# manikya7022/Continual-Learning-for-Dynamic-Video-Quality-Enhancement

Hardware: AMD Instinct MI355X
Metric: train frames/sec (2x SR, T=3, 540p->1080p) (higher is better)
Workload: dtype bf16

## Files before the change

### continual-learning-for-dynamic-video-quality-enhancement_amd/csrc/conv_bf16.hip

```cpp
#include "conv_common.h"

namespace nvq {

#ifdef NVQ_DEBUG_TOOLS
static int g_debug_mode = 0;
void set_conv_debug_mode(int m) { g_debug_mode = m; }
#else
constexpr int g_debug_mode = 0;
#endif

constexpr int XSB = 48;

__device__ __forceinline__ __bf16 pack_bf16_elem(const float* __restrict__ w, int cout_w, int cin_w, int taps, int transpose,
                                                 int cout_keep, int NT, int nkc, long idx) {
    const int stride = ws_stride_halfs(taps, NT);
    long t = idx % stride;
    const long slab = idx / stride;
    if (t >= (long)taps * 4 * NT * 8) return (__bf16)0.f;
    const int j = t & 7; t >>= 3;
    const int n = t % NT; t /= NT;
    const int g = t & 3; t >>= 2;
    const int tap = (int)t;
    const int kc = slab % nkc;
    const int cz = (int)(slab / nkc);
// ... 651 lines not shown
#pragma unroll
                for (int xh = 0; xh < 2; ++xh) {
#pragma unroll
                    for (int cb = 0; cb < NB; ++cb)
                        acc[cb][xh] = __builtin_amdgcn_mfma_f32_16x16x32_bf16(wa[cb], lo[xh], acc[cb][xh], 0, 0, 0);
                    if (same_dx) nhi[xh] = ldP(dy + 2, xh, ndx);
                    else if (!last) nlo[xh] = ldP(0, xh, ndx);
                }
#pragma unroll
                for (int xh = 0; xh < 2; ++xh) {
#pragma unroll
                    for (int cb = 0; cb < NB; ++cb)
                        acc[cb][2 + xh] = __builtin_amdgcn_mfma_f32_16x16x32_bf16(wa[cb], hi[xh], acc[cb][2 + xh], 0, 0, 0);
                    if (same_dx) nlo[xh] = hi[xh];
                    else if (!last) nhi[xh] = ldP(1, xh, ndx);
                }
                if (!last) {
#pragma unroll
                    for (int xh = 0; xh < 2; ++xh) { lo[xh] = nlo[xh]; hi[xh] = nhi[xh]; }
#pragma unroll
                    for (int cb = 0; cb < NB; ++cb) wa[cb] = wn[cb];
                }
            }
        }
        __syncthreads();
        reinterpret_cast<u32x4*>(wl)[rtid] = lr;
        __bf16* t4 = ws;
        if (!(dbg & 32)) conv_epilogue<NB>(d3, acc, n, ty, tx, 0, w4, c, g, vec3, TH, t4 + w4 * (2 * TW * T4S));
        __syncthreads();
        if (!(dbg & 32)) {
            __bf16* o16 = reinterpret_cast<__bf16*>(d3.out);
            const __bf16* stage = t4 + w4 * (2 * TW * T4S);
#pragma unroll
            for (int k = 0; k < 4; ++k) {
                const int item = lane + k * 64;
                const int px = item >> 2, piece = item & 3;
                const int gy = ty * TH + 2 * w4 + (px >> 5), gx = tx * TW + (px & 31);
                if (gy < H && gx < W)
                    *reinterpret_cast<u32x4*>(o16 + ((size_t)(n * H + gy) * W + gx) * d3.out_ld + d3.out_coff + 8 * piece) =
                        *reinterpret_cast<const u32x4*>(stage + px * T4S + 8 * piece);
            }
        }
        __syncthreads();
        return;
    }
    f32x4 lacc[NBL][4];
#pragma unroll
    for (int b = 0; b < 4; ++b)
#pragma unroll
        for (int a = 0; a < NBL; ++a) lacc[a][b] = (f32x4){0.f, 0.f, 0.f, 0.f};
    unsigned xoff[XPER];
    bool xok[XPER];
#pragma unroll
    for (int k = 0; k < XPER; ++k) xoff[k] = halo_off(rtid + k * 256, xok[k]);
    u32x4 xr[XPER];
    auto fetch = [&](int kc) {
        int sh;
        const unsigned o0 = chunk_off(kc, sh);
#pragma unroll
        for (int k = 0; k < XPER; ++k) xr[k] = *reinterpret_cast<const u32x4*>(in16 + ((xoff[k] << sh) + o0));
    };
    auto ldL = [&](int cb) -> bf16x8 {
        return *reinterpret_cast<const bf16x8*>(wl + (g * NTL + cb * 16 + c) * 8);
    };
    if (!(dbg & 64)) fetch(0);
    for (int kc = 0; kc < nkc; ++kc) {
        __syncthreads();
        if (!(dbg & 8)) {
            const u32x4 z = {0u, 0u, 0u, 0u};
#pragma unroll
            for (int k = 0; k < XPER; ++k) {
                const int item = rtid + k * 256;
                *reinterpret_cast<u32x4*>(xs + (item >> 2) * XSB + 8 * (item & 3)) = xok[k] ? xr[k] : z;
            }
        }
        __syncthreads();
        if (kc + 1 < nkc && !(dbg & 4)) fetch(kc + 1);
        if (dbg & 2) continue;
        bf16x8 px[4];
        px[0] = ldP(1, 0, 1); px[1] = ldP(1, 1, 1); px[2] = ldP(2, 0, 1); px[3] = ldP(2, 1, 1);
#pragma unroll
        for (int cb = 0; cb < NBL; ++cb) {
            const bf16x8 wf = ldL(cb);
#pragma unroll
            for (int pb = 0; pb < 4; ++pb)
                lacc[cb][pb] = __builtin_amdgcn_mfma_f32_16x16x32_bf16(wf, px[pb], lacc[cb][pb], 0, 0, 0);
        }
    }
    bool okp[4];
    uint2 rr[4][NBL];
    float4 bb[NBL];
    const __bf16* r16 = reinterpret_cast<const __bf16*>(dl.res) + dl.res_coff;
    auto res_load = [&](int pb) {
        const int gy = ty * TH + 2 * w4 + (pb >> 1), gx = tx * TW + (pb & 1) * 16 + c;
        okp[pb] = gy < H && gx < W;
        const unsigned off = okp[pb] ? ((unsigned)(n * H + gy) * (unsigned)W + gx) * (unsigned)dl.res_ld + 4u * g : 0u;
#pragma unroll
        for (int cb = 0; cb < NBL; ++cb) rr[pb][cb] = *reinterpret_cast<const uint2*>(r16 + (off + cb * 16u));
    };
    if (!(dbg & 128)) { res_load(0); res_load(1); }
    __syncthreads();
    __syncthreads();
    {
        const __bf16* t4 = ws;
#pragma unroll
        for (int cb = 0; cb < NBL; ++cb) {
            const bf16x8 wf = ldL(cb);
#pragma unroll
            for (int pb = 0; pb < 4; ++pb) {
                const int px = (2 * w4 + (pb >> 1)) * TW + (pb & 1) * 16 + c;
                const bf16x8 yf = *reinterpret_cast<const bf16x8*>(t4 + px * T4S + 8 * g);
                lacc[cb][pb] = __builtin_amdgcn_mfma_f32_16x16x32_bf16(wf, yf, lacc[cb][pb], 0, 0, 0);
            }
        }
    }
    if (!(dbg & 128)) { res_load(2); res_load(3); }
#pragma unroll
    for (int cb = 0; cb < NBL; ++cb) bb[cb] = ld4(dl.bias + cb * 16 + 4 * g);
    __syncthreads();
    __bf16* stage = lds + w4 * (2 * TW * STAGE_PX64);
#pragma unroll
    for (int pb = 0; pb < 4; ++pb) {
        if (!okp[pb]) continue;
#pragma unroll
        for (int cb = 0; cb < NBL; ++cb) {
            float v[4] = {lacc[cb][pb][0] + bb[cb].x, lacc[cb][pb][1] + bb[cb].y, lacc[cb][pb][2] + bb[cb].z,
                          lacc[cb][pb][3] + bb[cb].w};
            {
#pragma clang fp contract(off)
                v[0] = v[0] * dl.alpha + __uint_as_float(rr[pb][cb].x << 16);
                v[1] = v[1] * dl.alpha + __uint_as_float(rr[pb][cb].x & 0xffff0000u);
                v[2] = v[2] * dl.alpha + __uint_as_float(rr[pb][cb].y << 16);
                v[3] = v[3] * dl.alpha + __uint_as_float(rr[pb][cb].y & 0xffff0000u);
            }
            *reinterpret_cast<bf16x4*>(stage + ((pb >> 1) * TW + (pb & 1) * 16 + c) * STAGE_PX64 + cb * 16 + 4 * g) =
                (bf16x4){(__bf16)v[0], (__bf16)v[1], (__bf16)v[2], (__bf16)v[3]};
        }
    }
    __builtin_amdgcn_fence(__ATOMIC_RELEASE, "wavefront");
    __builtin_amdgcn_wave_barrier();
    if (dbg & 16) return;
    __bf16* o16 = reinterpret_cast<__bf16*>(dl.out);
#pragma unroll
    for (int k = 0; k < 8; ++k) {
        const int item = lane + k * 64;
        const int px = item >> 3, piece = item & 7;
        const int gy = ty * TH + 2 * w4 + (px >> 5), gx = tx * TW + (px & 31);
        if (gy < H && gx < W)
            *reinterpret_cast<u32x4*>(o16 + ((size_t)(n * H + gy) * W + gx) * dl.out_ld + dl.out_coff + 8 * piece) =
                *reinterpret_cast<const u32x4*>(stage + px * STAGE_PX64 + 8 * piece);
    }
}

template <int KS, bool XB, bool YB, int CIC, int COC = 32>
__global__ __launch_bounds__(256, 2) void wgrad_bf16_kernel(const nvq_wgrad_desc d, int tilesX, int tilesY,
                                                             int ntiles, int nci32, int nco) {
    static_assert(CIC == 32 || (CIC == 64 && XB), "64-channel chunks need bf16 x");
    static_assert(COC == 32 || (COC == 64 && CIC == 64 && YB && KS == 1), "64-co chunks: 1x1, bf16 x and dy");
    constexpr int HALO = KS / 2;
    constexpr int TAPS = KS * KS;
    constexpr int HW_ = TW + 2 * HALO;
    constexpr int HH_ = TH + 2 * HALO;
    constexpr int NPIX = HW_ * HH_;
    constexpr int XSX = CIC == 64 ? 80 : XSB;
    constexpr int XPP = (XB ? 4 : 8) * (CIC / 32);
    constexpr int YSX = COC == 64 ? 80 : XSB;
    constexpr int YPP = (YB ? 4 : 8) * (COC / 32);
    constexpr int XCH = CIC / XPP, YCH = COC / YPP;
    constexpr int XITEMS = NPIX * XPP;
    constexpr int XPER = (XITEMS + 255) / 256;
    constexpr int YPER = TH * TW * YPP / 256;
    constexpr int NCO = (CIC == 64 ? 2 : 1) * (COC / 32);
    __shared__ __attribute__((aligned(16))) __bf16 lds[NPIX * XSX + TH * TW * YSX];
    __bf16* xs = lds;
    __bf16* dys = lds + NPIX * XSX;

    const int tid = threadIdx.x;
    const int lane = tid & 63;
    const int wave = tid >> 6;
    const int r = lane & 15;
    const int g = lane >> 4;
    const int q = r >> 2, p = r & 3;
    const int cib = CIC == 64 ? wave : wave >> 1;
    const int cob0 = CIC == 64 ? 0 : (wave & 1);
    const int cic = blockIdx.y, coc = blockIdx.z;
    const int H = d.h, W = d.w;
    const float* x32 = d.x + d.x_coff;
    const __bf16* x16 = reinterpret_cast<const __bf16*>(d.x) + d.x_coff;
    const float* dy32 = d.dy + d.dy_coff;
    const __bf16* dy16 = reinterpret_cast<const __bf16*>(d.dy) + d.dy_coff;

    f32x4 acc[NCO][TAPS];
#pragma unroll
    for (int a = 0; a < NCO; ++a)
#pragma unroll
        for (int t = 0; t < TAPS; ++t) acc[a][t] = (f32x4){0.f, 0.f, 0.f, 0.f};

    u32x4 xr[XPER], yr[YPER];
    float4 bsumA = make_float4(0.f, 0.f, 0.f, 0.f), bsumB = bsumA;
    const int xq = XCH * (tid & (XPP - 1));
    const int yq = YCH * (tid & (YPP - 1));
    const bool xch_ok = cic * CIC + xq < d.cin;
    const int xch = cic * CIC + xq;
    const bool xlead = !d.x_plane || xch < d.x_ld;
    const unsigned xmul = xlead ? d.x_ld : 32;
    const size_t xbase = xlead ? (size_t)xch : (size_t)(xch >> 5) * d.x_plane + (xch & 31);
    const int ych = coc * COC + yq;
    const bool ych_ok = ych < d.cout;
    unsigned xmask = 0, ymask = 0;
    auto fetch = [&](int tile) {
        int bt = xcd_tile(tile, ntiles);
        const int tx = bt % tilesX; bt /= tilesX;
        const int ty = bt % tilesY;
        const int n = bt / tilesY;
        xmask = 0; ymask = 0;
#pragma unroll
        for (int k = 0; k < XPER; ++k) {
            const int item = tid + k * 256;
            const int hp = item / XPP;
            const int hy = hp / HW_, hx = hp - hy * HW_;
            const int gy = ty * TH + hy - HALO, gx = tx * TW + hx - HALO;
            const bool ok = item < XITEMS && gy >= 0 && gy < H && gx >= 0 && gx < W && xch_ok;
            xmask |= (ok ? 1u : 0u) << k;
            const size_t off = ok ? ((size_t)(n * H + gy) * W + gx) * xmul + xbase : 0;
            if constexpr (XB) xr[k] = *reinterpret_cast<const u32x4*>(x16 + off);
            else xr[k] = *reinterpret_cast<const u32x4*>(x32 + off);
        }
#pragma unroll
        for (int k = 0; k < YPER; ++k) {
            const int item = tid + k * 256;
            const int pp = item / YPP;
            const int py = pp / TW, px = pp - py * TW;
            const int gy = ty * TH + py, gx = tx * TW + px;
            const bool ok = gy < H && gx < W && ych_ok;
            ymask |= (ok ? 1u : 0u) << k;
            const size_t off = ok ? ((size_t)(n * H + gy) * W + gx) * d.dy_ld + ych : 0;
            if constexpr (YB) yr[k] = *reinterpret_cast<const u32x4*>(dy16 + off);
            else yr[k] = *reinterpret_cast<const u32x4*>(dy32 + off);
        }
    };
    auto commit = [&]() {
        const u32x4 z = {0u, 0u, 0u, 0u};
#pragma unroll
        for (int k = 0; k < XPER; ++k) {
            const int item = tid + k * 256;
            if (item < XITEMS) {
                const u32x4 v = (xmask >> k) & 1 ? xr[k] : z;
                __bf16* dst = xs + (item / XPP) * XSX + XCH * (item & (XPP - 1));
                if constexpr (XB) *reinterpret_cast<u32x4*>(dst) = v;
                else *reinterpret_cast<bf16x4*>(dst) = cvt4(as_f4(v));
            }
        }
#pragma unroll
        for (int k = 0; k < YPER; ++k) {
            const int item = tid + k * 256;
            const u32x4 v = (ymask >> k) & 1 ? yr[k] : z;
            __bf16* dst = dys + (item / YPP) * YSX + YCH * (item & (YPP - 1));
            if constexpr (YB) {
                *reinterpret_cast<u32x4*>(dst) = v;
                bsumA.x += bf_lo(v[0]); bsumA.y += bf_hi(v[0]); bsumA.z += bf_lo(v[1]); bsumA.w += bf_hi(v[1]);
                bsumB.x += bf_lo(v[2]); bsumB.y += bf_hi(v[2]); bsumB.z += bf_lo(v[3]); bsumB.w += bf_hi(v[3]);
            } else {
                const float4 f = as_f4(v);
                *reinterpret_cast<bf16x4*>(dst) = cvt4(f);
                bsumA.x += f.x; bsumA.y += f.y; bsumA.z += f.z; bsumA.w += f.w;
            }
        }
    };
    const bool idle = cic * CIC + cib * 16 >= d.cin_w;
    typedef s16x4 __attribute__((address_space(3))) * lds_s16x4_ptr;
    auto tr_read = [&](const __bf16* base, int stride, int pix, int chblock) -> s16x4 {
        return __builtin_amdgcn_ds_read_tr16_b64_v4i16((lds_s16x4_ptr)(base + (pix + q) * stride + chblock * 16 + 4 * p));
    };

    int tile = blockIdx.x;
    if (tile < ntiles) fetch(tile);
    for (; tile < ntiles; tile += gridDim.x) {
        __syncthreads();
        commit();
        __syncthreads();
        if (tile + (int)gridDim.x < ntiles) fetch(tile + gridDim.x);
        if (idle) continue;
#pragma unroll 2
        for (int py = 0; py < TH; ++py) {
            bf16x8 bfrag[NCO];
#pragma unroll
            for (int a = 0; a < NCO; ++a) {
                const s16x4 b0 = tr_read(dys, YSX, py * TW + 4 * g, cob0 + a);
                const s16x4 b1 = tr_read(dys, YSX, py * TW + 16 + 4 * g, cob0 + a);
                bfrag[a] = __builtin_bit_cast(bf16x8, __builtin_shufflevector(b0, b1, 0, 1, 2, 3, 4, 5, 6, 7));
            }
#pragma unroll
            for (int tap = 0; tap < TAPS; ++tap) {
                const int ddy = tap / KS, ddx = tap - ddy * KS;
                const int hp = (py + ddy) * HW_ + ddx;
                const s16x4 a0 = tr_read(xs, XSX, hp + 4 * g, cib);
                const s16x4 a1 = tr_read(xs, XSX, hp + 16 + 4 * g, cib);
                const bf16x8 afrag = __builtin_bit_cast(bf16x8, __builtin_shufflevector(a0, a1, 0, 1, 2, 3, 4, 5, 6, 7));
#pragma unroll
                for (int a = 0; a < NCO; ++a)
                    acc[a][tap] = __builtin_amdgcn_mfma_f32_16x16x32_bf16(afrag, bfrag[a], acc[a][tap], 0, 0, 0);
            }
        }
    }

    const int slab = cic * (CIC / 32) + (cib * 16) / 32;
    if (slab < nci32) {
        const int cil0 = (cib * 16) % 32;
#pragma unroll
        for (int a = 0; a < NCO; ++a) {
            const int coc32 = coc * (COC / 32) + (cob0 + a) / 2, cob = (cob0 + a) % 2;
            if (coc32 >= nco) continue;
            float* part = d.workspace + ((size_t)(blockIdx.x * nci32 + slab) * nco + coc32) * (TAPS * WG_C * WG_C);
#pragma unroll
            for (int tap = 0; tap < TAPS; ++tap)
#pragma unroll
                for (int e = 0; e < 4; ++e) part[(tap * WG_C + cil0 + 4 * g + e) * WG_C + cob * 16 + r] = acc[a][tap][e];
        }
    }

    if (cic == 0 && d.dbias != nullptr) {
        float* scratch = reinterpret_cast<float*>(lds);
        __syncthreads();
        st4(scratch + 8 * tid, bsumA);
        st4(scratch + 8 * tid + 4, bsumB);
        __syncthreads();
        if (tid < COC) {
            const int piece = tid / YCH, e = tid % YCH;
            float s = 0.f;
            for (int k = 0; k < 256 / YPP; ++k) s += scratch[8 * (YPP * k + piece) + e];
            float* bp = d.workspace + (size_t)WGRAD_MAX_SLABS * 9 * WG_C * WG_C;
            const int coc32 = coc * (COC / 32) + tid / WG_C;
            if (coc32 < nco) bp[((size_t)blockIdx.x * nco + coc32) * WG_C + tid % WG_C] = s;
        }
    }
}

size_t pack_floats_bf16(int cout, int cin_store, int ksize) {
    const int NT = choose_nt(cout);
    const size_t ncz = (cout + NT - 1) / NT, nkc = (cin_store + KCB - 1) / KCB;
    return ncz * nkc * (size_t)ws_stride_halfs(ksize * ksize, NT) / 2;
}

int pack_bf16(const float* w, int cout_w, int cin_w, int ksize, int transpose, int cin_store, int cout_keep,
              float* wpack, hipStream_t s) {
    const int cout = transpose ? cout_keep : cout_w;
    const int NT = choose_nt(cout);
    const int ncz = (cout + NT - 1) / NT, nkc = (cin_store + KCB - 1) / KCB;
    const long total = (long)ncz * nkc * ws_stride_halfs(ksize * ksize, NT);
    int nblk = ceil_div(total, 256);
    if (nblk > 2048) nblk = 2048;
    hipLaunchKernelGGL(pack_bf16_kernel, dim3(nblk), dim3(256), 0, s, w, cout_w, cin_w, ksize * ksize, transpose,
                       cout_keep, NT, ncz, nkc, reinterpret_cast<__bf16*>(wpack));
    return check_launch("conv_pack_bf16");
}

PackJobDev pack_job_bf16(const nvq_pack_job& j) {
    const int cout = j.transpose ? j.cout_keep : j.cout_w;
    const int NT = choose_nt(cout);
    const int ncz = (cout + NT - 1) / NT, nkc = (j.cin_store + KCB - 1) / KCB;
    return PackJobDev{j.w, j.wpack, j.cout_w, j.cin_w, j.ksize * j.ksize, j.transpose, j.cout_keep, NT, ncz, nkc,
                      (long)ncz * nkc * ws_stride_halfs(j.ksize * j.ksize, NT)};
}

int pack_batch_bf16(const PackJobTable& t, int n, hipStream_t s) {
    hipLaunchKernelGGL(pack_batch_bf16_kernel, dim3(32, n), dim3(256), 0, s, t);
    return check_launch("conv_pack_batch(bf16)");
}

int conv_forward_bf16(const nvq_conv_desc& d, int vec_ok, hipStream_t s) {
    NVQ_REQUIRE((size_t)d.n * d.h * d.w * d.in_ld < ((size_t)1 << 32),
                "conv_forward(bf16): input tensor of %d x %d x %d x %d elements exceeds the 32-bit offsets of the kernels", d.n,
                d.h, d.w, d.in_ld);
    const int NT = choose_nt(d.cout);
    const int ncz = (d.cout_store + NT - 1) / NT;
    const int nkc = (d.cin + KCB - 1) / KCB;
    int tilesX = (d.w + TW - 1) / TW, tilesY = (d.h + TH - 1) / TH;
    const bool underfilled = tilesX * ((d.h + 2 * TH - 1) / (2 * TH)) < NVQ_SMALL_IMAGE_TILES;
    const int rows = d.tile_rows == 0 && underfilled ? 8 : d.tile_rows;
    if (d.ksize == 3 && NT == 32 && d.in_bf16 && d.h >= 2 * TH && vec_ok &&
        (rows == 162 || rows == 164 || (rows == 0 && d.cin <= 128)))
        return conv_forward_m32(d, rows == 164 ? 4 : 2, g_debug_mode & 15, s);
    if (d.ksize == 3 && NT == 32 && d.in_bf16 && d.h >= 2 * TH && rows != 8) {
        tilesY = (d.h + 2 * TH - 1) / (2 * TH);
        const dim3 grid8((unsigned)((long)tilesX * tilesY * d.n), ncz);
        hipLaunchKernelGGL((conv_bf16_kernel<2, 3, true, 8>), grid8, dim3(512), 0, s, d, tilesX, tilesY, nkc, vec_ok,
                           g_debug_mode & 3, TailArgs{});
        return check_launch("conv_forward_bf16");
    }
    if (d.ksize == 3 && NT == 64 && d.in_bf16 && (d.tile_rows == 264 || d.tile_rows == 265)) {
        NVQ_REQUIRE(vec_ok && d.out_bf16 && d.cout_store % 64 == 0 && d.cin % 8 == 0,
                    "conv_forward: tile_rows 264 / 265 need bf16 output and a multiple of 64 stored channels");
        return conv_forward_m32(d, d.tile_rows == 264 ? 64 : 65, g_debug_mode & 3, s);
    }
    if (d.ksize == 3 && NT == 64 && d.in_bf16 && d.tile_rows != 8) {
        const dim3 grid8((unsigned)((long)tilesX * tilesY * d.n), ncz);
        hipLaunchKernelGGL((conv_bf16_kernel<2, 3, true, 8, 2>), grid8, dim3(512), 0, s, d, tilesX, tilesY, nkc, vec_ok,
                           g_debug_mode & 3, TailArgs{});
        return check_launch("conv_forward_bf16");
    }
    const dim3 grid((unsigned)((long)tilesX * tilesY * d.n), ncz);
#define NVQ_LAUNCH_CONVB(NB, KS)                                                                                        \
    do {                                                                                                                 \
        if (d.in_bf16)                                                                                                   \
            hipLaunchKernelGGL((conv_bf16_kernel<NB, KS, true>), grid, dim3(256), 0, s, d, tilesX, tilesY, nkc, vec_ok, g_debug_mode & 3, TailArgs{});   \
        else                                                                                                             \
            hipLaunchKernelGGL((conv_bf16_kernel<NB, KS, false>), grid, dim3(256), 0, s, d, tilesX, tilesY, nkc, vec_ok, g_debug_mode & 3, TailArgs{});  \
    } while (0)
    if (d.ksize == 3) {
        if (NT == 16) NVQ_LAUNCH_CONVB(1, 3);
        else if (NT == 32) NVQ_LAUNCH_CONVB(2, 3);
        else NVQ_LAUNCH_CONVB(4, 3);
    } else {
        if (NT == 16) NVQ_LAUNCH_CONVB(1, 1);
        else if (NT == 32) NVQ_LAUNCH_CONVB(2, 1);
        else NVQ_LAUNCH_CONVB(4, 1);
    }
#undef NVQ_LAUNCH_CONVB
    return check_launch("conv_forward_bf16");
}

int upsampler_tail_bf16(const nvq_conv_desc& d, const float* frames, int T, int t_center, int Cimg, int s, float* out,
                        unsigned char* pass, hipStream_t st) {
    NVQ_REQUIRE((size_t)d.n * d.h * d.w * d.in_ld < ((size_t)1 << 32), "upsampler_tail: tensor exceeds 32-bit offsets");
    const int tilesX = (d.w + TW - 1) / TW, tilesY = (d.h + TH - 1) / TH;
    const int nkc = (d.cin + KCB - 1) / KCB;
    const dim3 grid((unsigned)((long)tilesX * tilesY * d.n), 1);
    const TailArgs t{frames, out, pass, T, t_center, Cimg};
    if (s == 2 && Cimg * 4 <= 16)
        hipLaunchKernelGGL((conv_bf16_kernel<1, 3, true, 4, 1, 2>), grid, dim3(256), 0, st, d, tilesX, tilesY, nkc, 0, 0, t);
    else if (s == 3 && Cimg * 9 <= 32)
        hipLaunchKernelGGL((conv_bf16_kernel<2, 3, true, 4, 1, 3>), grid, dim3(256), 0, st, d, tilesX, tilesY, nkc, 0, 0, t);
    else if (s == 4 && Cimg * 16 <= 64)
        hipLaunchKernelGGL((conv_bf16_kernel<4, 3, true, 4, 1, 4>), grid, dim3(256), 0, st, d, tilesX, tilesY, nkc, 0, 0, t);
    else
        NVQ_REQUIRE(false, "upsampler_tail: scale %d with %d image channels", s, Cimg);
    return check_launch("upsampler_tail_forward");
}

void conv_occupancy_bf16(int* out) {
    (void)hipOccupancyMaxActiveBlocksPerMultiprocessor(&out[0], conv_bf16_kernel<2, 3, true, 8>, 512, 0);
    (void)hipOccupancyMaxActiveBlocksPerMultiprocessor(&out[1], conv_bf16_kernel<2, 3, true, 8, 2>, 512, 0);
    (void)hipOccupancyMaxActiveBlocksPerMultiprocessor(&out[2], conv_bf16_kernel<4, 3, true, 4>, 256, 0);
    (void)hipOccupancyMaxActiveBlocksPerMultiprocessor(&out[3], rdb_tail_kernel, 256, 0);
    (void)hipOccupancyMaxActiveBlocksPerMultiprocessor(&out[4], wgrad_bf16_kernel<3, true, true, 64, 32>, 256, 0);
    (void)hipOccupancyMaxActiveBlocksPerMultiprocessor(&out[5], conv_bf16_kernel<2, 3, true, 4>, 256, 0);
}

int rdb_tail_bf16(const nvq_conv_desc& d3, const nvq_conv_desc& dl, int vec3, int vecl, hipStream_t s) {
    NVQ_REQUIRE((size_t)d3.n * d3.h * d3.w * d3.in_ld < ((size_t)1 << 32) &&
                    (!dl.res || (size_t)dl.n * dl.h * dl.w * dl.res_ld < ((size_t)1 << 32)),
                "rdb_tail_forward: tensor exceeds 32-bit offsets");
    const int tilesX = (d3.w + TW - 1) / TW, tilesY = (d3.h + TH - 1) / TH;
    const int nkc = d3.cin / KCB;
    const bool usual = dl.out_bf16 && dl.bias && dl.res && dl.res_bf16 && dl.res_cmax >= 64 && !dl.out2 && !dl.relu && vecl;
    if ((d3.tile_rows & 255) == 4 || !usual)
        hipLaunchKernelGGL(rdb_tail_kernel, dim3((unsigned)((long)tilesX * tilesY * d3.n)), dim3(256), 0, s, d3, dl, tilesX,
                           tilesY, nkc, vec3, vecl);
    else
        hipLaunchKernelGGL(rdb_tail8_kernel, dim3((unsigned)((long)tilesX * tilesY * d3.n)), dim3(512), 0, s, d3, dl, tilesX,
                           tilesY, nkc, vec3, vecl);
    return check_launch("rdb_tail_forward");
}

int conv_wgrad_bf16(const nvq_wgrad_desc& d, int nsplit, int nci, int nco, int tilesX, int tilesY, int ntiles,
                    hipStream_t s) {
    if ((d.variant & 15) != 1 && wgrad_m32_takes(d)) return conv_wgrad_m32(d, s);
    NVQ_REQUIRE((d.variant & 15) != 2, "conv_wgrad: variant 2 (all-input-channel kernel) does not take %d -> %d channels, ksize %d",
                d.cin, d.cout, d.ksize);
    const bool wide = d.x_bf16 && d.dy_bf16 && d.cin_w >= 64;
    const int ncig = wide ? (nci + 1) / 2 : nci;
    if (wide) {
        nsplit = WGRAD_MAX_WG / (ncig * nco);
        if (nsplit < 1) nsplit = 1;
        if (nsplit > ntiles) nsplit = ntiles;
        if (nsplit >= 8) nsplit &= ~7;
    }
    NVQ_REQUIRE((size_t)nsplit * nci * nco * d.ksize * d.ksize <= (size_t)WGRAD_MAX_SLABS * 9,
                "conv_wgrad(bf16): %d splits x %d x %d chunks exceed the workspace", nsplit, nci, nco);
    if (wide && d.ksize == 1 && d.cout >= 64) {
        const int nco64 = (nco + 1) / 2;
        nsplit = WGRAD_MAX_WG / (ncig * nco64);
        const int cap = WGRAD_MAX_SLABS * 9 / (nci * nco * d.ksize * d.ksize);
        if (nsplit > cap) nsplit = cap;
        if (nsplit < 1) nsplit = 1;
        if (nsplit > ntiles) nsplit = ntiles;
        if (nsplit >= 8) nsplit &= ~7;
        NVQ_REQUIRE((size_t)nsplit * nci * nco * d.ksize * d.ksize <= (size_t)WGRAD_MAX_SLABS * 9,
                    "conv_wgrad(bf16, 64 co): %d splits x %d x %d chunks exceed the workspace", nsplit, nci, nco);
        hipLaunchKernelGGL((wgrad_bf16_kernel<1, true, true, 64, 64>), dim3(nsplit, ncig, nco64), dim3(256), 0, s, d, tilesX,
                           tilesY, ntiles, nci, nco);
        return nsplit;
    }
    const dim3 grid(nsplit, ncig, nco);
#define NVQ_LAUNCH_WG(KS, XB, YB, CIC) \
    hipLaunchKernelGGL((wgrad_bf16_kernel<KS, XB, YB, CIC>), grid, dim3(256), 0, s, d, tilesX, tilesY, ntiles, nci, nco)
    if (d.ksize == 3) {
        if (wide) NVQ_LAUNCH_WG(3, true, true, 64);
        else if (d.x_bf16 && d.dy_bf16) NVQ_LAUNCH_WG(3, true, true, 32);
        else if (d.x_bf16) NVQ_LAUNCH_WG(3, true, false, 32);
        else if (d.dy_bf16) NVQ_LAUNCH_WG(3, false, true, 32);
        else NVQ_LAUNCH_WG(3, false, false, 32);
    } else {
        if (wide) NVQ_LAUNCH_WG(1, true, true, 64);
        else if (d.x_bf16 && d.dy_bf16) NVQ_LAUNCH_WG(1, true, true, 32);
        else if (d.x_bf16) NVQ_LAUNCH_WG(1, true, false, 32);
        else if (d.dy_bf16) NVQ_LAUNCH_WG(1, false, true, 32);
        else NVQ_LAUNCH_WG(1, false, false, 32);
    }
#undef NVQ_LAUNCH_WG
    return nsplit;
}

}
```

### continual-learning-for-dynamic-video-quality-enhancement_amd/csrc/conv_igemm.hip

```cpp
#include "conv_common.h"
#include "flat.h"

namespace nvq {

constexpr int KC = 16;
constexpr int XS_LD = 20;

__device__ __forceinline__ float pack_f32_elem(const float* __restrict__ w, int cout_w, int cin_w, int taps, int transpose,
                                               int cout_keep, int NT, int nkc, long idx) {
    long t = idx;
    const int j = t & 3; t >>= 2;
    const int n = t % NT; t /= NT;
    const int g = t & 3; t >>= 2;
    const int tap = t % taps; t /= taps;
    const int kc = t % nkc; t /= nkc;
    const int cz = (int)t;
    const int co = cz * NT + n;
    const int ch = kc * KC + 4 * g + j;
    float v = 0.f;
    if (!transpose) {
        if (co < cout_w && ch < cin_w) v = w[((long)co * cin_w + ch) * taps + tap];
    } else {
        if (co < cout_keep && ch < cout_w) v = w[((long)ch * cin_w + co) * taps + (taps - 1 - tap)];
    }
// ... 550 lines not shown
#ifdef NVQ_DEBUG_TOOLS
int nvq_debug_set_conv_mode(int mode) { set_conv_debug_mode(mode); return NVQ_OK; }
int nvq_debug_conv_occupancy(int* out6) { conv_occupancy_bf16(out6); return NVQ_OK; }
#endif

size_t nvq_sizeof_conv_desc(void) { return sizeof(nvq_conv_desc); }
size_t nvq_sizeof_wgrad_desc(void) { return sizeof(nvq_wgrad_desc); }
size_t nvq_sizeof_wgrad_reduce_job(void) { return sizeof(nvq_wgrad_reduce_job); }

static int epilogue_vec_ok(const nvq_conv_desc& d) {
    int v = d.out_ld % 4 == 0 && d.out_coff % 4 == 0 && d.cout_store % 4 == 0 && aligned16(d.out) && (d.cout % 4 == 0 || !d.bias);
    if (d.bias && !aligned16(d.bias)) v = 0;
    if (d.out2 && !(d.out2_ld % 4 == 0 && d.out2_coff % 4 == 0 && aligned16(d.out2))) v = 0;
    if (d.res && !(d.res_ld % 4 == 0 && d.res_coff % 4 == 0 && d.res_cmax % 4 == 0 && aligned16(d.res))) v = 0;
    if (d.mask && !(d.mask_ld % 4 == 0 && d.mask_coff % 4 == 0 && d.mask_c0 % 4 == 0 && d.mask_c1 % 4 == 0 && aligned16(d.mask))) v = 0;
    return v;
}

static bool planar_input_ok(const nvq_conv_desc& d) {
    return d.math == NVQ_MATH_BF16 && d.in_bf16 && d.cin % 32 == 0 && d.in_coff == 0 &&
           (d.in_ld == 32 || d.in_ld == 64 || d.in_ld == 128) && d.in_ld <= d.cin &&
           (size_t)d.in_plane == (size_t)d.n * d.h * d.w * 32 && (size_t)(d.cin / 32) * d.in_plane < ((size_t)1 << 32);
}

int nvq_rdb_tail_forward(const nvq_conv_desc* d3p, const nvq_conv_desc* dlp, void* stream) {
    const nvq_conv_desc d3 = *d3p, dl = *dlp;
    NVQ_REQUIRE(d3.math == NVQ_MATH_BF16 && dl.math == NVQ_MATH_BF16 && d3.in_bf16 && dl.in_bf16,
                "rdb_tail_forward: NVQ_MATH_BF16 with a bf16 concat buffer only");
    NVQ_REQUIRE(d3.ksize == 3 && dl.ksize == 1 && d3.cout == 32 && d3.cout_store == 32 && dl.cout == 64 && dl.cout_store == 64,
                "rdb_tail_forward: 3x3 -> 32 channels followed by 1x1 -> 64 channels");
    NVQ_REQUIRE(d3.cin % 32 == 0 && dl.cin == d3.cin + 32 && dl.in == d3.in && dl.in_ld == d3.in_ld && dl.in_coff == d3.in_coff &&
                    dl.in_plane == d3.in_plane && d3.out_bf16,
                "rdb_tail_forward: both convs must read the same buffer");
    if (d3.in_plane) {
        NVQ_REQUIRE(planar_input_ok(d3) && d3.out_ld == 32 && d3.out_coff == 0 &&
                        (const char*)d3.out == (const char*)d3.in + (size_t)(d3.cin / 32) * d3.in_plane * 2,
                    "rdb_tail_forward: the 3x3 layer must write plane cin/32 of the slice-planar buffer both convs read");
    } else {
        NVQ_REQUIRE(d3.out == (float*)d3.in && d3.out_ld == d3.in_ld && d3.out_coff == d3.in_coff + d3.cin,
                    "rdb_tail_forward: the 3x3 layer must write channels [cin, cin+32) of the buffer both convs read");
    }
    NVQ_REQUIRE(d3.n == dl.n && d3.h == dl.h && d3.w == dl.w && d3.n > 0 && d3.h > 0 && d3.w > 0, "rdb_tail_forward: shapes");
    NVQ_REQUIRE(d3.in_ld % 8 == 0 && d3.in_coff % 8 == 0 && aligned16(d3.in) && aligned16(d3.wpack) && aligned16(dl.wpack),
                "rdb_tail_forward: alignment");
    NVQ_REQUIRE(!d3.res && !d3.out2 && !d3.mask && !d3.accumulate && d3.bits_mode != 2 && !dl.bits_mode && !dl.mask && !dl.accumulate,
                "rdb_tail_forward: unsupported epilogue");
    NVQ_REQUIRE(!d3.bias || aligned16(d3.bias), "rdb_tail_forward: bias alignment");
    const int vec3 = epilogue_vec_ok(d3), vecl = epilogue_vec_ok(dl);
    NVQ_REQUIRE(vec3 && vecl, "rdb_tail_forward: the epilogues must be 16-byte addressable");
    NVQ_REQUIRE(!d3.bits_mode || d3.bits, "rdb_tail_forward: bits");
    return rdb_tail_bf16(d3, dl, vec3, vecl, (hipStream_t)stream);
}

int nvq_upsampler_tail_forward(const nvq_conv_desc* dp, const float* frames, int T, int t_center, int Cimg, int s, float* out,
                               uint8_t* pass, void* stream) {
    const nvq_conv_desc d = *dp;
    NVQ_REQUIRE(d.math == NVQ_MATH_BF16 && d.in_bf16 && d.ksize == 3, "upsampler_tail_forward: NVQ_MATH_BF16, bf16 input, 3x3 only");
    NVQ_REQUIRE(d.cin > 0 && d.cin % 8 == 0 && d.in_ld % 8 == 0 && d.in_coff % 8 == 0 && aligned16(d.in) && !d.in_plane,
                "upsampler_tail_forward: input must be a 16-byte addressable bf16 slice");
    NVQ_REQUIRE(s >= 2 && s <= 4 && Cimg >= 1 && d.cout == Cimg * s * s && t_center >= 0 && t_center < T && frames && out && pass,
                "upsampler_tail_forward: cout %d for %d image channels at scale %d", d.cout, Cimg, s);
    NVQ_REQUIRE(aligned16(d.wpack) && d.n > 0 && d.h > 0 && d.w > 0 && d.center_cin == 0, "upsampler_tail_forward: args");
    return upsampler_tail_bf16(d, frames, T, t_center, Cimg, s, out, pass, (hipStream_t)stream);
}

int nvq_conv_forward(const nvq_conv_desc* dp, void* stream) {
    const nvq_conv_desc d = *dp;
    NVQ_REQUIRE(d.math == NVQ_MATH_F32 || d.math == NVQ_MATH_BF16, "conv_forward: math mode %d", d.math);
    NVQ_REQUIRE(d.ksize == 1 || d.ksize == 3, "conv_forward: ksize %d", d.ksize);
    NVQ_REQUIRE(d.cin > 0 && d.cin % 4 == 0 && d.in_ld % 4 == 0 && d.in_coff % 4 == 0 &&
                    aligned16(d.in),
                "conv_forward: input must be 16-byte addressable (cin %d ld %d coff %d)", d.cin,
                d.in_ld, d.in_coff);
    NVQ_REQUIRE(d.cout > 0 && d.cout_store >= d.cout, "conv_forward: cout %d store %d", d.cout,
                d.cout_store);
    NVQ_REQUIRE(d.out_coff + d.cout_store <= d.out_ld, "conv_forward: output slice exceeds ld");
    NVQ_REQUIRE(aligned16(d.wpack), "conv_forward: wpack alignment");
    NVQ_REQUIRE(d.n > 0 && d.h > 0 && d.w > 0, "conv_forward: empty shape");
    NVQ_REQUIRE(!d.in_plane || planar_input_ok(d),
                "conv_forward: a slice-planar input needs NVQ_MATH_BF16, bf16 storage, cin %% 32 == 0, in_coff 0, in_ld in "
                "{32, 64, 128} and in_plane = n*h*w*32 (cin %d ld %d plane %u)", d.cin, d.in_ld, d.in_plane);
    NVQ_REQUIRE(d.center_cin >= 0 && d.center_cin % 32 == 0 && d.center_cin <= d.cin && (d.center_cin == 0 || d.ksize == 3),
                "conv_forward: center_cin %d (3x3 only, multiple of 32, <= cin %d)", d.center_cin, d.cin);
    const int NT = choose_nt(d.cout);
    const int ncz = (d.cout_store + NT - 1) / NT;
    NVQ_REQUIRE(ncz == (d.cout + NT - 1) / NT, "conv_forward: cout_store %d crosses a pack chunk", d.cout_store);
    const int nkc = (d.cin + KC - 1) / KC;
    const int tilesX = (d.w + TW - 1) / TW, tilesY = (d.h + TH - 1) / TH;
    int vec_ok = d.out_ld % 4 == 0 && d.out_coff % 4 == 0 && d.cout_store % 4 == 0 && aligned16(d.out) &&
                 (d.cout % 4 == 0 || !d.bias);
    if (d.bias && !aligned16(d.bias)) vec_ok = 0;
    if (d.bits_mode != 0)
        NVQ_REQUIRE((d.bits_mode == 1 || d.bits_mode == 2) && d.bits && d.math == NVQ_MATH_BF16 &&
                        ((NT <= 32 && ncz == 1) || (NT == 64 && d.ksize == 3 && d.in_bf16 && d.tile_rows != 8)) &&
                        (d.bits_words > 0 ? d.bits_words : 1) * 32 >= d.cout_store && vec_ok && !d.mask && !d.res &&
                        !d.accumulate && !d.out2,
                    "conv_forward: bit masks need NVQ_MATH_BF16, a plain vector epilogue and cout <= 32 (or a 3x3 conv of a bf16 "
                    "input), bits_words * 32 >= cout_store");
    if (d.out2 && !(d.out2_ld % 4 == 0 && d.out2_coff % 4 == 0 && aligned16(d.out2))) vec_ok = 0;
    if (d.res && !(d.res_ld % 4 == 0 && d.res_coff % 4 == 0 && d.res_cmax % 4 == 0 && aligned16(d.res))) vec_ok = 0;
    if (d.mask && !(d.mask_ld % 4 == 0 && d.mask_coff % 4 == 0 && d.mask_c0 % 4 == 0 &&
                    d.mask_c1 % 4 == 0 && aligned16(d.mask)))
        vec_ok = 0;
    const dim3 grid((unsigned)((long)tilesX * tilesY * d.n), ncz);
    hipStream_t s = (hipStream_t)stream;
    const int epi_bf16 = d.out_bf16 | d.out2_bf16 | d.res_bf16 | d.mask_bf16;
    NVQ_REQUIRE(!(epi_bf16 | d.in_bf16) || d.math == NVQ_MATH_BF16, "conv_forward: bf16 tensors need NVQ_MATH_BF16");
    NVQ_REQUIRE(!epi_bf16 || vec_ok, "conv_forward: bf16 output / residual / mask tensors need 4-channel aligned slices");
    NVQ_REQUIRE(!d.in_bf16 || (d.cin % 8 == 0 && d.in_ld % 8 == 0 && d.in_coff % 8 == 0),
                "conv_forward: a bf16 input needs cin, ld, coff %% 8 == 0 (cin %d ld %d coff %d)", d.cin, d.in_ld, d.in_coff);
    if (d.math == NVQ_MATH_BF16) return conv_forward_bf16(d, vec_ok, s);
    NVQ_REQUIRE((size_t)d.n * d.h * d.w * d.in_ld < ((size_t)1 << 32),
                "conv_forward: input tensor of %d x %d x %d x %d elements exceeds the 32-bit offsets of the kernels", d.n, d.h, d.w,
                d.in_ld);
    int gs = 1;
    while (gs * 2 <= NT / 16 && (long)grid.x * grid.y * gs * 2 <= 512) gs *= 2;
    const dim3 gridz(grid.x, grid.y, gs);
#define NVQ_LAUNCH_CONV(NB, KS, GS) \
    hipLaunchKernelGGL((conv_f32_kernel<NB, KS, GS>), gridz, dim3(256), 0, s, d, tilesX, tilesY, nkc, vec_ok)
#define NVQ_LAUNCH_CONV_KS(KS)                                       \
    do {                                                             \
        if (NT == 16) NVQ_LAUNCH_CONV(1, KS, 1);                     \
        else if (NT == 32) {                                         \
            if (gs == 1) NVQ_LAUNCH_CONV(2, KS, 1);                  \
            else NVQ_LAUNCH_CONV(1, KS, 2);                          \
        } else {                                                     \
            if (gs == 1) NVQ_LAUNCH_CONV(4, KS, 1);                  \
            else if (gs == 2) NVQ_LAUNCH_CONV(2, KS, 2);             \
            else NVQ_LAUNCH_CONV(1, KS, 4);                          \
        }                                                            \
    } while (0)
    if (d.ksize == 3) NVQ_LAUNCH_CONV_KS(3);
    else NVQ_LAUNCH_CONV_KS(1);
#undef NVQ_LAUNCH_CONV_KS
#undef NVQ_LAUNCH_CONV
    return check_launch("conv_forward");
}

size_t nvq_wgrad_workspace_bytes(void) {
    return (size_t)WGRAD_MAX_SLABS * 9 * WG_C * WG_C * sizeof(float) + (size_t)512 * 256 * sizeof(float);
}

static int wgrad_partial(const nvq_wgrad_desc* dp, nvq_wgrad_reduce_job* job, void* stream) {
    const nvq_wgrad_desc d = *dp;
    NVQ_REQUIRE(d.math == NVQ_MATH_F32 || d.math == NVQ_MATH_BF16, "conv_wgrad: math mode %d", d.math);
    NVQ_REQUIRE(d.ksize == 1 || d.ksize == 3, "conv_wgrad: ksize %d", d.ksize);
    NVQ_REQUIRE(d.cin % 4 == 0 && d.x_ld % 4 == 0 && d.x_coff % 4 == 0 && aligned16(d.x),
                "conv_wgrad: x must be 16-byte addressable");
    NVQ_REQUIRE(d.dy_ld % 4 == 0 && d.dy_coff % 4 == 0 && aligned16(d.dy),
                "conv_wgrad: dy must be 16-byte addressable");
    NVQ_REQUIRE(d.cin_w > 0 && d.cin_w <= d.cin && d.cout > 0, "conv_wgrad: channels");
    NVQ_REQUIRE(!(d.x_bf16 | d.dy_bf16) || d.math == NVQ_MATH_BF16, "conv_wgrad: bf16 tensors need NVQ_MATH_BF16");
    NVQ_REQUIRE(!d.x_bf16 || (d.cin % 8 == 0 && d.x_ld % 8 == 0 && d.x_coff % 8 == 0), "conv_wgrad: bf16 x alignment");
    NVQ_REQUIRE(!d.dy_bf16 || (d.cout % 8 == 0 && d.dy_ld % 8 == 0 && d.dy_coff % 8 == 0), "conv_wgrad: bf16 dy alignment");
    NVQ_REQUIRE(d.math != NVQ_MATH_BF16 || d.dy_coff + ((d.cout + 3) & ~3) <= d.dy_ld,
                "conv_wgrad(bf16): the dy slice must be readable up to a multiple of 4 channels");
    NVQ_REQUIRE(d.workspace_bytes >= nvq_wgrad_workspace_bytes(), "conv_wgrad: workspace too small");
    NVQ_REQUIRE(!d.x_plane || (d.math == NVQ_MATH_BF16 && d.x_bf16 && d.x_coff == 0 && d.cin % 32 == 0 &&
                               (d.x_ld == 32 || d.x_ld == 64 || d.x_ld == 128) && d.x_ld <= d.cin &&
                               (size_t)d.x_plane == (size_t)d.n * d.h * d.w * 32),
                "conv_wgrad: a slice-planar x needs NVQ_MATH_BF16, bf16 storage, cin %% 32 == 0, x_coff 0, x_ld in {32, 64, 128} "
                "and x_plane = n*h*w*32");
    const int taps = d.ksize * d.ksize;
    const int nci = (d.cin_w + WG_C - 1) / WG_C, nco = (d.cout + WG_C - 1) / WG_C;
    const int tilesX = (d.w + TW - 1) / TW, tilesY = (d.h + TH - 1) / TH;
    const int ntiles = tilesX * tilesY * d.n;
    int nsplit = WGRAD_MAX_WG / (nci * nco);
    if (nsplit < 1) nsplit = 1;
    if (nsplit > ntiles) nsplit = ntiles;
    if (nsplit >= 8) nsplit &= ~7;
    NVQ_REQUIRE((size_t)nsplit * nci * nco * taps * WG_C * WG_C * sizeof(float) <= d.workspace_bytes,
                "conv_wgrad: %d x %d channel chunks exceed the workspace", nci, nco);
    hipStream_t s = (hipStream_t)stream;
    const dim3 grid(nsplit, nci, nco);
    int rc;
    if (d.math == NVQ_MATH_BF16) {
        const int used = conv_wgrad_bf16(d, nsplit, nci, nco, tilesX, tilesY, ntiles, s);
        if (used < 0) return used;
        rc = check_launch("conv_wgrad_bf16");
        if (used > 0) nsplit = used;
    } else {
        if (d.ksize == 3)
            hipLaunchKernelGGL((wgrad_f32_kernel<3>), grid, dim3(256), 0, s, d, tilesX, tilesY, ntiles, nci, nco);
        else
            hipLaunchKernelGGL((wgrad_f32_kernel<1>), grid, dim3(256), 0, s, d, tilesX, tilesY, ntiles, nci, nco);
        rc = check_launch("conv_wgrad");
    }
    if (rc) return rc;
    *job = nvq_wgrad_reduce_job{d.workspace, d.workspace + (size_t)WGRAD_MAX_SLABS * 9 * WG_C * WG_C, d.dw, d.dbias, nsplit, nci,
                                nco, taps, d.cout, d.cin_w, d.alpha, d.accumulate};
    return NVQ_OK;
}

int nvq_conv_wgrad(const nvq_wgrad_desc* dp, void* stream) {
    nvq_wgrad_reduce_job j;
    const int rc = wgrad_partial(dp, &j, stream);
    if (rc) return rc;
    return launch_wgrad_reduce_bias(j.part, j.nsplit, j.nci, j.nco, j.taps, j.cout, j.cin_w, j.alpha, j.accumulate, j.dw,
                                    j.bias_part, j.dbias, (hipStream_t)stream);
}

int nvq_conv_wgrad_partial(const nvq_wgrad_desc* dp, nvq_wgrad_reduce_job* job, void* stream) {
    NVQ_REQUIRE(job != nullptr, "conv_wgrad_partial: job");
    return wgrad_partial(dp, job, stream);
}

int nvq_wgrad_reduce_batch(const nvq_wgrad_reduce_job* jobs, int n, void* stream) {
    NVQ_REQUIRE(n >= 0 && (n == 0 || jobs != nullptr), "wgrad_reduce_batch: jobs");
    for (int i = 0; i < n; ++i)
        NVQ_REQUIRE(jobs[i].part && jobs[i].dw && jobs[i].nsplit > 0 && jobs[i].nci > 0 && jobs[i].nco > 0 &&
                        (jobs[i].taps == 1 || jobs[i].taps == 9) && (!jobs[i].dbias || jobs[i].bias_part),
                    "wgrad_reduce_batch: job %d is not one nvq_conv_wgrad_partial filled in", i);
    for (int i0 = 0; i0 < n; i0 += WR_MAX_JOBS) {
        const int m = n - i0 < WR_MAX_JOBS ? n - i0 : WR_MAX_JOBS;
        WgradReduceTable t;
        long need = 1;
        for (int i = 0; i < m; ++i) {
            t.j[i] = jobs[i0 + i];
            const long total = (long)t.j[i].nci * t.j[i].nco * t.j[i].taps * WG_C * WG_C;
            long b = ceil_div(total, WR_E);
            if (b > 1024) b = 1024;
            b += t.j[i].dbias ? ceil_div(t.j[i].cout, 4) : 0;
            if (b > need) need = b;
        }
        hipLaunchKernelGGL(wgrad_reduce_batch_kernel, dim3((unsigned)need, (unsigned)m), dim3(256), 0, (hipStream_t)stream, t);
        const int rc = check_launch("wgrad_reduce_batch");
        if (rc) return rc;
    }
    return NVQ_OK;
}


int nvq_colsum(const float* x, int x_ld, int x_coff, int C, long npix, float alpha, float* out,
               float* workspace, size_t workspace_bytes, int accumulate, void* stream) {
    return colsum_impl(x, x_ld, x_coff, C, npix, alpha, out, workspace, workspace_bytes, accumulate,
                       (hipStream_t)stream);
}

}
```

Measured before the change: 77.53.

## Add eight-wave 64x64-channel 3x3 bf16 weight-gradient kernel

Adds an eight-wave (512-thread) variant of the bf16 wgrad kernel for 3x3 convolutions. Each block covers 64 input and 64 output channels, with each wave owning a 16-channel input block and half the output channels. The inner loop is restructured to walk halo rows, reusing each x fragment across all three vertical taps and caching dy fragments per row. The goal is fewer LDS reads and staging passes per MFMA and fewer blocks over the channel grid. Split counts are recomputed for the larger blocks, and the bf16 dy alignment checks are relaxed. Risks include higher register pressure from the per-row fragment cache and lower parallelism from fewer splits.

Result: faster. 78.73, median of 6 (+1.5%).

```diff
diff --git a/continual-learning-for-dynamic-video-quality-enhancement_amd/csrc/conv_bf16.hip b/continual-learning-for-dynamic-video-quality-enhancement_amd/csrc/conv_bf16.hip
--- a/continual-learning-for-dynamic-video-quality-enhancement_amd/csrc/conv_bf16.hip
+++ b/continual-learning-for-dynamic-video-quality-enhancement_amd/csrc/conv_bf16.hip
@@ -827,11 +827,14 @@
     }
 }
 
-template <int KS, bool XB, bool YB, int CIC, int COC = 32>
-__global__ __launch_bounds__(256, 2) void wgrad_bf16_kernel(const nvq_wgrad_desc d, int tilesX, int tilesY,
-                                                             int ntiles, int nci32, int nco) {
+template <int KS, bool XB, bool YB, int CIC, int COC = 32, int NW = 4>
+__global__ __launch_bounds__(64 * NW, 2) void wgrad_bf16_kernel(const nvq_wgrad_desc d, int tilesX, int tilesY,
+                                                                int ntiles, int nci32, int nco) {
     static_assert(CIC == 32 || (CIC == 64 && XB), "64-channel chunks need bf16 x");
-    static_assert(COC == 32 || (COC == 64 && CIC == 64 && YB && KS == 1), "64-co chunks: 1x1, bf16 x and dy");
+    static_assert(COC == 32 || (COC == 64 && CIC == 64 && YB && (KS == 1 || NW == 8)),
+                  "64-co chunks: bf16 x and dy; 3x3 with eight waves");
+    static_assert(NW == 4 || (NW == 8 && KS == 3 && COC == 64), "eight waves: the 3x3 64-co form");
+    constexpr int NTHR = 64 * NW;
     constexpr int HALO = KS / 2;
     constexpr int TAPS = KS * KS;
     constexpr int HW_ = TW + 2 * HALO;
@@ -843,21 +846,21 @@
     constexpr int YPP = (YB ? 4 : 8) * (COC / 32);
     constexpr int XCH = CIC / XPP, YCH = COC / YPP;
     constexpr int XITEMS = NPIX * XPP;
-    constexpr int XPER = (XITEMS + 255) / 256;
-    constexpr int YPER = TH * TW * YPP / 256;
-    constexpr int NCO = (CIC == 64 ? 2 : 1) * (COC / 32);
+    constexpr int XPER = (XITEMS + NTHR - 1) / NTHR;
+    constexpr int YPER = TH * TW * YPP / NTHR;
+    constexpr int NCO = (CIC == 64 ? 2 : 1) * (COC / 32) / (NW / 4);
     __shared__ __attribute__((aligned(16))) __bf16 lds[NPIX * XSX + TH * TW * YSX];
     __bf16* xs = lds;
     __bf16* dys = lds + NPIX * XSX;
 
     const int tid = threadIdx.x;
     const int lane = tid & 63;
-    const int wave = tid >> 6;
+    const int wave = NW == 8 ? __builtin_amdgcn_readfirstlane(tid >> 6) : tid >> 6;
     const int r = lane & 15;
     const int g = lane >> 4;
     const int q = r >> 2, p = r & 3;
-    const int cib = CIC == 64 ? wave : wave >> 1;
-    const int cob0 = CIC == 64 ? 0 : (wave & 1);
+    const int cib = NW == 8 ? wave & 3 : (CIC == 64 ? wave : wave >> 1);
+    const int cob0 = NW == 8 ? (wave >> 2) * NCO : (CIC == 64 ? 0 : (wave & 1));
     const int cic = blockIdx.y, coc = blockIdx.z;
     const int H = d.h, W = d.w;
     const float* x32 = d.x + d.x_coff;
@@ -891,7 +894,7 @@
         xmask = 0; ymask = 0;
 #pragma unroll
         for (int k = 0; k < XPER; ++k) {
-            const int item = tid + k * 256;
+            const int item = tid + k * NTHR;
             const int hp = item / XPP;
             const int hy = hp / HW_, hx = hp - hy * HW_;
             const int gy = ty * TH + hy - HALO, gx = tx * TW + hx - HALO;
@@ -903,7 +906,7 @@
         }
 #pragma unroll
         for (int k = 0; k < YPER; ++k) {
-            const int item = tid + k * 256;
+            const int item = tid + k * NTHR;
             const int pp = item / YPP;
             const int py = pp / TW, px = pp - py * TW;
             const int gy = ty * TH + py, gx = tx * TW + px;
@@ -918,7 +921,7 @@
         const u32x4 z = {0u, 0u, 0u, 0u};
 #pragma unroll
         for (int k = 0; k < XPER; ++k) {
-            const int item = tid + k * 256;
+            const int item = tid + k * NTHR;
             if (item < XITEMS) {
                 const u32x4 v = (xmask >> k) & 1 ? xr[k] : z;
                 __bf16* dst = xs + (item / XPP) * XSX + XCH * (item & (XPP - 1));
@@ -928,7 +931,7 @@
         }
 #pragma unroll
         for (int k = 0; k < YPER; ++k) {
-            const int item = tid + k * 256;
+            const int item = tid + k * NTHR;
             const u32x4 v = (ymask >> k) & 1 ? yr[k] : z;
             __bf16* dst = dys + (item / YPP) * YSX + YCH * (item & (YPP - 1));
             if constexpr (YB) {
@@ -942,7 +945,8 @@
             }
         }
     };
-    const bool idle = cic * CIC + cib * 16 >= d.cin_w;
+    const bool co_dead = NW == 8 && coc * COC + cob0 * 16 >= d.cout;
+    const bool idle = cic * CIC + cib * 16 >= d.cin_w || co_dead;
     typedef s16x4 __attribute__((address_space(3))) * lds_s16x4_ptr;
     auto tr_read = [&](const __bf16* base, int stride, int pix, int chblock) -> s16x4 {
         return __builtin_amdgcn_ds_read_tr16_b64_v4i16((lds_s16x4_ptr)(base + (pix + q) * stride + chblock * 16 + 4 * p));
@@ -956,6 +960,36 @@
         __syncthreads();
         if (tile + (int)gridDim.x < ntiles) fetch(tile + gridDim.x);
         if (idle) continue;
+        if constexpr (NW == 8) {
+            bf16x8 bfrag[TH][NCO];
+#pragma unroll
+            for (int hy = 0; hy < HH_; ++hy) {
+                if (hy < TH) {
+#pragma unroll
+                    for (int a = 0; a < NCO; ++a) {
+                        const s16x4 b0 = tr_read(dys, YSX, hy * TW + 4 * g, cob0 + a);
+                        const s16x4 b1 = tr_read(dys, YSX, hy * TW + 16 + 4 * g, cob0 + a);
+                        bfrag[hy][a] = __builtin_bit_cast(bf16x8, __builtin_shufflevector(b0, b1, 0, 1, 2, 3, 4, 5, 6, 7));
+                    }
+                }
+#pragma unroll
+                for (int ddx = 0; ddx < KS; ++ddx) {
+                    const s16x4 a0 = tr_read(xs, XSX, hy * HW_ + ddx + 4 * g, cib);
+                    const s16x4 a1 = tr_read(xs, XSX, hy * HW_ + ddx + 16 + 4 * g, cib);
+                    const bf16x8 afrag = __builtin_bit_cast(bf16x8, __builtin_shufflevector(a0, a1, 0, 1, 2, 3, 4, 5, 6, 7));
+#pragma unroll
+                    for (int ddy = 0; ddy < KS; ++ddy) {
+                        const int py = hy - ddy;
+                        if (py < 0 || py >= TH) continue;
+#pragma unroll
+                        for (int a = 0; a < NCO; ++a)
+                            acc[a][ddy * KS + ddx] =
+                                __builtin_amdgcn_mfma_f32_16x16x32_bf16(afrag, bfrag[py][a], acc[a][ddy * KS + ddx], 0, 0, 0);
+                    }
+                }
+            }
+            continue;
+        }
 #pragma unroll 2
         for (int py = 0; py < TH; ++py) {
             bf16x8 bfrag[NCO];
@@ -1003,7 +1037,7 @@
         if (tid < COC) {
             const int piece = tid / YCH, e = tid % YCH;
             float s = 0.f;
-            for (int k = 0; k < 256 / YPP; ++k) s += scratch[8 * (YPP * k + piece) + e];
+            for (int k = 0; k < NTHR / YPP; ++k) s += scratch[8 * (YPP * k + piece) + e];
             float* bp = d.workspace + (size_t)WGRAD_MAX_SLABS * 9 * WG_C * WG_C;
             const int coc32 = coc * (COC / 32) + tid / WG_C;
             if (coc32 < nco) bp[((size_t)blockIdx.x * nco + coc32) * WG_C + tid % WG_C] = s;
@@ -1140,9 +1174,24 @@
 
 int conv_wgrad_bf16(const nvq_wgrad_desc& d, int nsplit, int nci, int nco, int tilesX, int tilesY, int ntiles,
                     hipStream_t s) {
-    if ((d.variant & 15) != 1 && wgrad_m32_takes(d)) return conv_wgrad_m32(d, s);
-    NVQ_REQUIRE((d.variant & 15) != 2, "conv_wgrad: variant 2 (all-input-channel kernel) does not take %d -> %d channels, ksize %d",
+    const int variant = d.variant & 15;
+    if (variant != 1 && variant != 3 && wgrad_m32_takes(d)) return conv_wgrad_m32(d, s);
+    NVQ_REQUIRE(variant != 2, "conv_wgrad: variant 2 (all-input-channel kernel) does not take %d -> %d channels, ksize %d",
                 d.cin, d.cout, d.ksize);
+    if (d.ksize == 3 && d.x_bf16 && d.dy_bf16 && d.cout > 32 && d.cin_w > 32 && variant != 3) {
+        const int ncig = (nci + 1) / 2, nco64 = (nco + 1) / 2;
+        nsplit = WGRAD_MAX_WG / 2 / (ncig * nco64);
+        const int cap = WGRAD_MAX_SLABS / (nci * nco);
+        if (nsplit > cap) nsplit = cap;
+        if (nsplit < 1) nsplit = 1;
+        if (nsplit > ntiles) nsplit = ntiles;
+        if (nsplit >= 8) nsplit &= ~7;
+        NVQ_REQUIRE((size_t)nsplit * nci * nco * 9 <= (size_t)WGRAD_MAX_SLABS * 9,
+                    "conv_wgrad(bf16, 3x3, 64 co): %d splits x %d x %d chunks exceed the workspace", nsplit, nci, nco);
+        hipLaunchKernelGGL((wgrad_bf16_kernel<3, true, true, 64, 64, 8>), dim3(nsplit, ncig, nco64), dim3(512), 0, s, d, tilesX,
+                           tilesY, ntiles, nci, nco);
+        return nsplit;
+    }
     const bool wide = d.x_bf16 && d.dy_bf16 && d.cin_w >= 64;
     const int ncig = wide ? (nci + 1) / 2 : nci;
     if (wide) {
diff --git a/continual-learning-for-dynamic-video-quality-enhancement_amd/csrc/conv_igemm.hip b/continual-learning-for-dynamic-video-quality-enhancement_amd/csrc/conv_igemm.hip
--- a/continual-learning-for-dynamic-video-quality-enhancement_amd/csrc/conv_igemm.hip
+++ b/continual-learning-for-dynamic-video-quality-enhancement_amd/csrc/conv_igemm.hip
@@ -726,9 +726,9 @@
     NVQ_REQUIRE(d.cin_w > 0 && d.cin_w <= d.cin && d.cout > 0, "conv_wgrad: channels");
     NVQ_REQUIRE(!(d.x_bf16 | d.dy_bf16) || d.math == NVQ_MATH_BF16, "conv_wgrad: bf16 tensors need NVQ_MATH_BF16");
     NVQ_REQUIRE(!d.x_bf16 || (d.cin % 8 == 0 && d.x_ld % 8 == 0 && d.x_coff % 8 == 0), "conv_wgrad: bf16 x alignment");
-    NVQ_REQUIRE(!d.dy_bf16 || (d.cout % 8 == 0 && d.dy_ld % 8 == 0 && d.dy_coff % 8 == 0), "conv_wgrad: bf16 dy alignment");
-    NVQ_REQUIRE(d.math != NVQ_MATH_BF16 || d.dy_coff + ((d.cout + 3) & ~3) <= d.dy_ld,
-                "conv_wgrad(bf16): the dy slice must be readable up to a multiple of 4 channels");
+    NVQ_REQUIRE(!d.dy_bf16 || (d.dy_ld % 8 == 0 && d.dy_coff % 8 == 0), "conv_wgrad: bf16 dy alignment");
+    NVQ_REQUIRE(d.math != NVQ_MATH_BF16 || d.dy_coff + ((d.cout + (d.dy_bf16 ? 7 : 3)) & (d.dy_bf16 ? ~7 : ~3)) <= d.dy_ld,
+                "conv_wgrad(bf16): the dy slice must be readable up to a multiple of 4 (fp32) / 8 (bf16) channels");
     NVQ_REQUIRE(d.workspace_bytes >= nvq_wgrad_workspace_bytes(), "conv_wgrad: workspace too small");
     NVQ_REQUIRE(!d.x_plane || (d.math == NVQ_MATH_BF16 && d.x_bf16 && d.x_coff == 0 && d.cin % 32 == 0 &&
                                (d.x_ld == 32 || d.x_ld == 64 || d.x_ld == 128) && d.x_ld <= d.cin &&
```
